# maelaubert/VulkanSift

Hardware: AMD Instinct MI355X
Metric: SIFT detect+match frames/sec (640x480, ~2k kp) (higher is better)
Workload: dtype f32

## Files before the change

### vulkansift_amd/csrc/hip/extract_tail.hip

```cpp
#include <hip/hip_runtime.h>
#include <stdint.h>

#include "extrema_refine.h"
#include "multi.h"
#include "records.h"
#include "vksift_hip.h"
#include "wave.h"

namespace
{

constexpr uint32_t TAIL_SPT = 2;
constexpr uint32_t TAIL_LIST = 4096;

template <bool F16, bool BUF>
__global__ void __launch_bounds__(1024) __attribute__((amdgpu_waves_per_eu(6, 8))) k_extract_tail(Multi<ExtremaArgs> m)
{
  __shared__ uint32_t s_list[TAIL_LIST];
  __shared__ uint32_t s_wtot[2][16];
  __shared__ uint32_t s_cnt[2][16];
  const VBlock vb = vblock(m);
  const ExtremaArgs &a = m.oct[vb.o];
  const int b = (int)vb.x;
  const uint32_t tid = threadIdx.x, NT = blockDim.x, nw = NT >> 6, lane = tid & 63u, wave = tid >> 6;
  constexpr unsigned EB = F16 ? 2u : 4u;
  const DogView d{(const float *)((const uint8_t *)a.gauss + (size_t)b * a.img_stride * EB), a.w, a.h, a.pitch, (size_t)a.plane_stride, a.S};
  const __amdgpu_buffer_rsrc_t rsrc = __builtin_amdgcn_make_buffer_rsrc((void *)d.base, 0, (int)((unsigned)(a.S + 3) * (unsigned)a.plane_stride * EB), 0x00020000);
  const RefineCtx c{a, 0u, 0u, d, rsrc, nullptr, nullptr, nullptr};
  const uint64_t *__restrict__ mask = a.seg_mask + (size_t)b * a.seg_img_stride;
  uint8_t *const feats = a.feats + (size_t)b * a.feat_img_stride;
  const uint32_t nsegs = a.nsegs, tile = NT * TAIL_SPT;

  uint32_t base = 0;
  uint32_t ncand = 0;
  uint32_t fill = 0;
  uint32_t rpar = 0;

  auto round = [&](uint32_t c0, uint32_t cnt) {
    KpRecord kp;
    bool ok = false;
    if (tid < cnt)
      ok = refine_candidate<F16, BUF>(c, s_list[c0 + tid], &kp);
    const unsigned long long bal = __ballot(ok);
    if (lane == 0)
      s_cnt[rpar][wave] = (uint32_t)__popcll(bal);
    __syncthreads();
    uint32_t rank = ballot_rank(bal, (int)lane), total = 0;
    for (uint32_t wv = 0; wv < nw; wv++)
    {
      const uint32_t n = s_cnt[rpar][wv];
      rank += wv < wave ? n : 0u;
      total += n;
    }
    const uint32_t idx = base + rank;
    if (ok && idx < a.cap)
      store_record((uint32_t *)(feats + (size_t)idx * VKSIFT_RECORD_BYTES), kp);
    base += total;
    rpar ^= 1u;
  };

  auto load_tile = [&](uint32_t t0, unsigned long long(&mk)[TAIL_SPT]) {
    const uint32_t i0 = t0 + TAIL_SPT * tid;
#pragma unroll
    for (uint32_t k = 0; k < TAIL_SPT; k++)
      mk[k] = i0 + k < nsegs ? mask[i0 + k] : 0ull;
  };

  unsigned long long cur[TAIL_SPT];
  uint32_t tpar = 0;
  for (uint32_t t0 = 0; t0 < nsegs; t0 += tile, tpar ^= 1u)
  {
    load_tile(t0, cur);
    uint32_t tsum = 0;
#pragma unroll
    for (uint32_t k = 0; k < TAIL_SPT; k++)
      tsum += (uint32_t)__popcll(cur[k]);
    const uint32_t incl = wave_scan_incl_u32(tsum, (int)lane);
    if (lane == 63u)
      s_wtot[tpar][wave] = incl;
    __syncthreads();
    uint32_t off = incl - tsum, T = 0;
    for (uint32_t wv = 0; wv < nw; wv++)
    {
      const uint32_t n = s_wtot[tpar][wv];
      off += wv < wave ? n : 0u;
      T += n;
    }
    const uint32_t valid = ncand >= a.cand_cap ? 0u : (T < a.cand_cap - ncand ? T : a.cand_cap - ncand);
    ncand += T;
    for (uint32_t w0 = 0; w0 < valid;)
    {
      const uint32_t room = TAIL_LIST - fill, hi = valid - w0 < room ? valid : w0 + room;
      if (off < hi && off + tsum > w0)
      {
        uint32_t pos = off;
#pragma unroll
        for (uint32_t k = 0; k < TAIL_SPT; k++)
        {
          unsigned long long mk = cur[k];
          if (mk == 0ull)
            continue;
          const uint32_t seg = t0 + TAIL_SPT * tid + k;
          const uint32_t row = seg / (uint32_t)a.nseg, segx = seg - row * (uint32_t)a.nseg;
          const uint32_t sz = row / (uint32_t)a.h, yy = row - sz * (uint32_t)a.h;
          const uint32_t head = (segx * 64u) | (yy << 14) | ((sz + 1u) << 28);
          while (mk)
          {
            const uint32_t bit = (uint32_t)__ffsll((long long)mk) - 1u;
            mk &= mk - 1ull;
            if (pos >= w0 && pos < hi)
              s_list[fill + (pos - w0)] = head + bit;
            pos++;
          }
        }
      }
      fill += hi - w0;
      w0 = hi;
      __syncthreads();
      const uint32_t nfull = fill - fill % NT, left = fill - nfull;
      for (uint32_t c0 = 0; c0 < nfull; c0 += NT)
        round(c0, NT);
      if (nfull != 0u && left != 0u)
      {
        if (tid < left)
          s_list[tid] = s_list[nfull + tid];
        __syncthreads();
      }
      fill = left;
    }
  }
  if (fill != 0u)
    round(0u, fill);
  if (tid == 0u)
  {
    a.cand_n[b] = ncand;
    a.found[(size_t)b * a.found_img_stride] = base;
  }
}

}

int extract_tail_launch(const ExtremaArgs *args, uint32_t n, uint32_t batch, bool f16, bool buf, bool small_wg, hipStream_t hs)
{
  Multi<ExtremaArgs> mt;
  mt.n = 0;
  for (uint32_t i = 0; i < n; i++)
    if (!multi_add(mt, args[i], batch, 1u, 1u))
      return (int)hipErrorInvalidValue;
  const dim3 grid(mt.start[mt.n]), block(mt.start[mt.n] < 512u && !small_wg ? 1024u : 512u);
  with_bool(f16, [&](auto F16) {
    with_bool(buf, [&](auto BUF) { hipLaunchKernelGGL((k_extract_tail<decltype(F16)::value, decltype(BUF)::value>), grid, block, 0, hs, mt); });
  });
  return (int)hipGetLastError();
}
```

### vulkansift_amd/csrc/hip/extrema.hip

```cpp
#include <hip/hip_runtime.h>
#include <type_traits>
#include <vector>
#include <stdint.h>
#include <stdlib.h>

#include "../detmath.h"
#include "extrema_refine.h"
#include "multi.h"
#include "records.h"
#include "vksift_hip.h"
#include "wave.h"

namespace
{

__device__ __forceinline__ float wave_shr1(float v, float edge)
{
  return __builtin_bit_cast(float, __builtin_amdgcn_update_dpp(__builtin_bit_cast(int, edge), __builtin_bit_cast(int, v), 0x138, 0xf, 0xf, false));
}
__device__ __forceinline__ float wave_shl1(float v, float edge)
{
  return __builtin_bit_cast(float, __builtin_amdgcn_update_dpp(__builtin_bit_cast(int, edge), __builtin_bit_cast(int, v), 0x130, 0xf, 0xf, false));
}

// ... 162 lines not shown
      const float vxh = fmax3(ho, hm, hn), vnh = fmin3(ho, hm, hn);
      const float Lx = wave_shr1(vxb, vxh), Ln = wave_shr1(vnb, vnh);
      const float Rx = wave_shl1(vxa, vxh), Rn = wave_shl1(vna, vnh);
      if (l >= 1 && l <= S)
      {
        ownxA[l - 1] = fmax3(Lx, vxb, fmax2(ao, an)), ownnA[l - 1] = fmin3(Ln, vnb, fmin2(ao, an));
        ownxB[l - 1] = fmax3(vxa, Rx, fmax2(bo, bn)), ownnB[l - 1] = fmin3(vna, Rn, fmin2(bo, bn));
      }
      fullxA[l] = fmax3(Lx, vxa, vxb), fullnA[l] = fmin3(Ln, vna, vnb);
      fullxB[l] = fmax3(vxa, vxb, Rx), fullnB[l] = fmin3(vna, vnb, Rn);
    }
#pragma unroll
    for (int sz = 0; sz < S; sz++)
    {
      const int l = sz + 1;
      const float ca = __uint_as_float(wv2[sm][l].x), cb = __uint_as_float(wv2[sm][l].y);
      const float nxa = fmax3(ownxA[sz], fullxA[l - 1], fullxA[l + 1]), nna = fmin3(ownnA[sz], fullnA[l - 1], fullnA[l + 1]);
      const float nxb = fmax3(ownxB[sz], fullxB[l - 1], fullxB[l + 1]), nnb = fmin3(ownnB[sz], fullnB[l - 1], fullnB[l + 1]);
      const unsigned long long ma = (__ballot(ca > nxa) | __ballot(ca < nna)) & __ballot(fabsf(ca) > pre) & colA;
      const unsigned long long mb = (__ballot(cb > nxb) | __ballot(cb < nnb)) & __ballot(fabsf(cb) > pre) & colB;
      if ((ma | mb) != 0ull)
      {
        const unsigned lo = odd ? (unsigned)mb : (unsigned)ma, hi = odd ? (unsigned)(mb >> 32) : (unsigned)(ma >> 32);
        const unsigned long long m0 = __ballot((lo >> half) & 1u), m1 = __ballot((hi >> half) & 1u);
        if (lane == 0)
        {
          const size_t base = ((size_t)sz * a.h + y) * a.nseg + (size_t)b * a.seg_img_stride;
          a.seg_mask[base + seg0] = m0;
          if (has_seg1)
            a.seg_mask[base + seg0 + 1] = m1;
        }
      }
    }
  };

  if (AHEAD >= 1)
    fetch_row(y0 - 1, std::integral_constant<int, 0>{});
  if (AHEAD >= 2)
    fetch_row(y0, std::integral_constant<int, 1 % NSLOT>{});
  int r = y0 - 1;
  for (;;)
  {
    phase(std::integral_constant<int, 0>{}, r);
    if (++r > y1)
      break;
    phase(std::integral_constant<int, 1>{}, r);
    if (++r > y1)
      break;
    phase(std::integral_constant<int, 2>{}, r);
    if (++r > y1)
      break;
    phase(std::integral_constant<int, 3>{}, r);
    if (++r > y1)
      break;
    if (NSLOT > 4)
    {
      phase(std::integral_constant<int, 4 % NSLOT>{}, r);
      if (++r > y1)
        break;
    }
  }
}

constexpr uint32_t SEG_CHUNK = 4096;

__global__ void __launch_bounds__(1024) k_segment_scan(Multi<ExtremaArgs> m)
{
  __shared__ uint32_t wave_tot[16];
  const VBlock vb = vblock(m);
  const ExtremaArgs &a = m.oct[vb.o];
  const int b = (int)vb.y;
  const uint64_t *__restrict__ mask = a.seg_mask + (size_t)b * a.seg_img_stride;
  uint32_t *__restrict__ off = a.seg_off + (size_t)b * a.seg_img_stride;
  uint32_t *__restrict__ chunk_tot = a.cand_flag;
  const uint64_t chunk_img_stride = a.cand_img_stride;
  const uint32_t n = a.nsegs;
  const int lane = threadIdx.x & 63, wave = threadIdx.x >> 6;
  const uint32_t i0 = vb.x * SEG_CHUNK + 4u * threadIdx.x;
  uint32_t p[4];
#pragma unroll
  for (int k = 0; k < 4; k++)
    p[k] = i0 + k < n ? (uint32_t)__popcll(mask[i0 + k]) : 0u;
  const uint32_t tsum = p[0] + p[1] + p[2] + p[3];
  const uint32_t incl = wave_scan_incl_u32(tsum, lane);
  if (lane == 63)
    wave_tot[wave] = incl;
  __syncthreads();
  uint32_t wave_base = 0, total = 0;
  for (int wv = 0; wv < 16; wv++)
  {
    if (wv < wave)
      wave_base += wave_tot[wv];
    total += wave_tot[wv];
  }
  uint32_t run = wave_base + incl - tsum;
#pragma unroll
  for (int k = 0; k < 4; k++)
  {
    if (i0 + k < n)
      off[i0 + k] = run;
    run += p[k];
  }
  if (threadIdx.x == 0)
    chunk_tot[(size_t)b * chunk_img_stride + vb.x] = total;
}


__global__ void __launch_bounds__(256) k_cand_list(Multi<ExtremaArgs> mu)
{
  const VBlock vb = vblock(mu);
  const ExtremaArgs &a = mu.oct[vb.o];
  const uint32_t seg = vb.x * 256 + threadIdx.x;
  const int b = (int)vb.y;
  const uint32_t *chunk_tot = a.cand_flag + (size_t)b * a.cand_img_stride;
  if (vb.x == 0 && threadIdx.x == 0)
  {
    uint32_t total = 0;
    for (uint32_t c = 0; c < a.nchunks; c++)
      total += chunk_tot[c];
    a.cand_n[b] = total;
    if (total == 0)
      a.found[(size_t)b * a.found_img_stride] = 0;
  }
  unsigned long long m = seg < a.nsegs ? a.seg_mask[seg + (size_t)b * a.seg_img_stride] : 0ull;
  if (__ballot(m != 0ull) == 0ull)
    return;
  uint32_t base = 0;
  for (uint32_t c = threadIdx.x & 63u, nc = (vb.x * 256u) / SEG_CHUNK; c < nc; c += 64u)
    base += chunk_tot[c];
  base = wave_sum_u32(base);
  if (m == 0ull)
    return;
  uint32_t pos = a.seg_off[seg + (size_t)b * a.seg_img_stride] + base;
  const uint32_t segx = seg % (uint32_t)a.nseg;
  const uint32_t yy = (seg / (uint32_t)a.nseg) % (uint32_t)a.h;
  const uint32_t sz = seg / ((uint32_t)a.nseg * (uint32_t)a.h);
  uint32_t *out = a.cand_xy + (size_t)b * a.cand_img_stride;
  while (m)
  {
    const int bit = __ffsll((long long)m) - 1;
    m &= m - 1;
    if (pos < a.cand_cap)
      out[pos] = (segx * 64u + (uint32_t)bit) | (yy << 14) | ((sz + 1u) << 28);
    pos++;
  }
}

template <bool F16, bool BUF>
__global__ void __launch_bounds__(256) k_refine_flags(Multi<ExtremaArgs> m)
{
  __shared__ uint32_t s_cnt[4];
  const VBlock vb = vblock(m);
  const RefineCtx c = refine_ctx<F16>(m.oct[vb.o], (int)vb.x);
  for (uint32_t chunk = vb.y; chunk < c.nch; chunk += vb.gy)
  {
    const uint32_t i = chunk * 256u + threadIdx.x;
    bool ok = false;
    if (i < c.n)
    {
      KpRecord kp;
      ok = refine_candidate<F16, BUF>(c, c.xy[i], &kp);
      c.flag[i] = ok ? 1u : 0u;
    }
    const unsigned long long bal = __ballot(ok);
    if ((threadIdx.x & 63) == 0)
      s_cnt[threadIdx.x >> 6] = (uint32_t)__popcll(bal);
    __syncthreads();
// ... 229 lines not shown
```

### vulkansift_amd/csrc/hip/features.hip

```cpp
#include <hip/hip_runtime.h>
#include <stdint.h>
#include <stdlib.h>
#include <type_traits>

#include "../detmath.h"
#include "features_math.h"
#include "multi.h"
#include "records.h"
#include "vksift_hip.h"
#include "wave.h"

namespace
{

struct FeatArgs
{
  const float *gauss;
  uint32_t fp16;
  int w, h, pitch;
  uint64_t plane_stride, img_stride;
  uint8_t *feats;
  uint64_t feat_img_stride;
  uint32_t cap;
  uint32_t *found;
// ... 128 lines not shown
            px -= box, py++;
          const float sdx = (rsx + (float)dx) - kh.scale_x;
          const float sdy = (rsy + (float)dy) - kh.scale_y;
          const float d2 = (sdx * sdx) + (sdy * sdy);
          if constexpr (decltype(INTERIOR)::value)
          {
            const unsigned v0 = (__umul24((unsigned)(cyi + dy - 1), (unsigned)g.pitch) + (unsigned)(cxi + dx - 1)) * 4u;
            accumulate(d2, tap_ld<F16>(kh.rs, v0 + 8u, pitch4), tap_ld<F16>(kh.rs, v0, pitch4), tap_ld<F16>(kh.rs, v0 + 4u, 2 * pitch4), tap_ld<F16>(kh.rs, v0 + 4u, 0));
          }
          else
          {
            const int gx = cxi + dx, gy = cyi + dy;
            if ((gx < 1 || gx >= (g.w - 1) || gy < 1 || gy >= (g.h - 1)) && (d2 > (float)(r * r)))
              continue;
            const bool xin = (unsigned)gx < (unsigned)g.w, yin = (unsigned)gy < (unsigned)g.h;
            const unsigned o0 = (__umul24((unsigned)gy, (unsigned)g.pitch) + (unsigned)gx) * 4u;
            const unsigned o_r = (yin && (unsigned)(gx + 1) < (unsigned)g.w) ? o0 + 4u : 0x80000000u;
            const unsigned o_l = (yin && (unsigned)(gx - 1) < (unsigned)g.w) ? o0 - 4u : 0x80000000u;
            const unsigned o_d = (xin && (unsigned)(gy + 1) < (unsigned)g.h) ? (__umul24((unsigned)(gy + 1), (unsigned)g.pitch) + (unsigned)gx) * 4u : 0x80000000u;
            const unsigned o_u = (xin && (unsigned)(gy - 1) < (unsigned)g.h) ? (__umul24((unsigned)(gy - 1), (unsigned)g.pitch) + (unsigned)gx) * 4u : 0x80000000u;
            accumulate(d2, tap_ld<F16>(kh.rs, o_r, 0), tap_ld<F16>(kh.rs, o_l, 0), tap_ld<F16>(kh.rs, o_d, 0), tap_ld<F16>(kh.rs, o_u, 0));
          }
        }
      };
      if (cxi - r >= 1 && cxi + r <= g.w - 2 && cyi - r >= 1 && cyi + r <= g.h - 2)
        window(std::true_type{});
      else
        window(std::false_type{});
    }
    __builtin_amdgcn_wave_barrier();
    {
      const int li = lane < 36 ? lane : 0;
      uint32_t hv = hist[li];
      const int lm = (li + 35) % 36, lp = (li + 1) % 36;
#pragma unroll
      for (int it = 0; it < 6; it++)
      {
        uint32_t hm = __shfl(hv, lm, 64), hp = __shfl(hv, lp, 64);
        hv = (uint32_t)dm_div_3((float)(hm + hv + hp));
      }
      uint32_t hm = __shfl(hv, lm, 64), hp = __shfl(hv, lp, 64);
      const uint32_t mx = wave_max_u32(lane < 36 ? hv : 0u);
      bool peak = lane < 36 && ((float)hv >= (0.8f * (float)mx)) && (hv > hm) && (hv > hp);
      unsigned long long pm = __ballot(peak);
      uint32_t npk = (uint32_t)__popcll(pm);
      if (peak)
      {
        uint32_t rank = ballot_rank(pm, lane);
        if (rank < a.max_keep)
        {
          uint32_t num = hm - hp;
          uint32_t den = hm - (2u * hv) + hp;
          float idx = (float)lane + 0.5f * ((float)num / (float)den);
          float ang = (idx + 0.5f) * (2.f * PI_F) / 36.f;
          a.ori_ang[((size_t)b * a.ori_img_stride + k) * VKSIFT_HIP_MAX_ORI + rank] = ang;
        }
      }
      if (lane == 0)
        a.ori_cnt[(size_t)b * a.ori_img_stride + k] = npk < a.max_keep ? npk : a.max_keep;
    }
    __builtin_amdgcn_wave_barrier();
  }
}

__global__ void __launch_bounds__(1024) k_orientation_finalize(Multi<FeatArgs> m)
{
  __shared__ uint32_t wave_tot[16];
  __shared__ uint32_t carry_s;
  const VBlock vb = vblock(m);
  const FeatArgs &a = m.oct[vb.o];
  const int b = (int)vb.x;
  const int lane = threadIdx.x & 63, wave = threadIdx.x >> 6;
  const ImageView g = image_view(a, b);
  const uint32_t *cnt = a.ori_cnt + (size_t)b * a.ori_img_stride;
  const float *ang = a.ori_ang + (size_t)b * a.ori_img_stride * VKSIFT_HIP_MAX_ORI;
  if (threadIdx.x == 0)
    carry_s = 0;
  __syncthreads();
  for (uint32_t base = 0; base < g.n; base += 1024)
  {
    uint32_t k = base + threadIdx.x;
    uint32_t c = k < g.n ? cnt[k] : 0u;
    uint32_t v = c > 1 ? c - 1 : 0u;
    const uint32_t incl = wave_scan_incl_u32(v, lane);
    if (lane == 63)
      wave_tot[wave] = incl;
    __syncthreads();
    uint32_t wave_base = 0;
    for (int wv = 0; wv < wave; wv++)
      wave_base += wave_tot[wv];
    uint32_t carry = carry_s;
    uint32_t excl = carry + wave_base + incl - v;
    if (k < g.n && c >= 1)
    {
      uint32_t *rec = (uint32_t *)(g.feats + (size_t)k * VKSIFT_RECORD_BYTES);
      rec[7] = __float_as_uint(ang[(size_t)k * VKSIFT_HIP_MAX_ORI]);
      for (uint32_t j = 1; j < c; j++)
      {
        uint32_t idx = g.found + excl + (j - 1);
        if (idx < a.cap)
        {
          uint32_t *dst = (uint32_t *)(g.feats + (size_t)idx * VKSIFT_RECORD_BYTES);
#pragma unroll
          for (int q = 0; q < (int)VKSIFT_RECORD_HEAD_WORDS; q++)
            dst[q] = rec[q];
          dst[7] = __float_as_uint(ang[(size_t)k * VKSIFT_HIP_MAX_ORI + j]);
        }
      }
    }
    __syncthreads();
    if (threadIdx.x == 1023)
      carry_s = carry + wave_base + incl;
    __syncthreads();
  }
  if (threadIdx.x == 0)
    a.found[(size_t)b * a.found_img_stride] = g.found + carry_s;
}

__device__ __forceinline__ int smod8(int v) { return v & 7; }

struct DescCtx
{
  __amdgpu_buffer_rsrc_t rs;
  int pitch, pitch4;
  float scale_x, scale_y, rsx, rsy, kcos, ksin, kori, fp, bin_scale;
  int dx0, dx1, dy0, dy1;
  float offx, offy, ia0, ia1;
};

struct DescSample
{
  float ox, oy, mag;
  float xb;
};

struct DescTaps
{
  float up, lf, rt, dn;
};

__device__ __forceinline__ unsigned desc_tap_base(const DescCtx &c, int cdx, int cdy)
{
  const int ix = (int)c.rsx + cdx, iy = (int)c.rsy + cdy;
  return (__umul24((unsigned)(iy - 1), (unsigned)c.pitch) + (unsigned)(ix - 1)) * 4u;
}

template <bool F16>
__device__ __forceinline__ DescTaps desc_taps(const DescCtx &c, unsigned v0)
{
  DescTaps t;
  t.up = tap_ld<F16>(c.rs, v0 + 4u, 0);
  t.lf = tap_ld<F16>(c.rs, v0, c.pitch4);
  t.rt = tap_ld<F16>(c.rs, v0 + 8u, c.pitch4);
  t.dn = tap_ld<F16>(c.rs, v0 + 4u, 2 * c.pitch4);
  return t;
}

typedef uint32_t u32x2_t __attribute__((ext_vector_type(2)));
typedef uint32_t u32x4_t __attribute__((ext_vector_type(4)));
__device__ __forceinline__ void desc_taps_pair(const DescCtx &c, unsigned v0, DescTaps &a, DescTaps &b)
{
  const u32x2_t up = __builtin_amdgcn_raw_buffer_load_b64(c.rs, v0 + 4u, 0, 0);
  const u32x4_t mid = __builtin_amdgcn_raw_buffer_load_b128(c.rs, v0, c.pitch4, 0);
  const u32x2_t dn = __builtin_amdgcn_raw_buffer_load_b64(c.rs, v0 + 4u, 2 * c.pitch4, 0);
  a.up = __uint_as_float(up.x), b.up = __uint_as_float(up.y);
  a.lf = __uint_as_float(mid.x), b.lf = __uint_as_float(mid.y);
  a.rt = __uint_as_float(mid.z), b.rt = __uint_as_float(mid.w);
  a.dn = __uint_as_float(dn.x), b.dn = __uint_as_float(dn.y);
}

template <bool INRANGE>
__device__ __forceinline__ DescSample desc_sample(const DescCtx &c, int cdx, int cdy, const DescTaps &t, bool *odd)
{
  const float es = -1.f / (2.f * 2 * 2);
  float sdx = (c.rsx + (float)cdx) - c.scale_x;
  float sdy = (c.rsy + (float)cdy) - c.scale_y;
  DescSample r;
  r.ox = c.kcos * sdx + c.ksin * sdy;
  r.oy = c.kcos * sdy - c.ksin * sdx;
  float gradX = 0.5f * (t.rt - t.lf);
  float gradY = 0.5f * (t.dn - t.up);
  float ori, root;
  grad_polar<INRANGE>(gradX, gradY, &ori, &root, odd);
  ori = wrap_2pi(ori);
  ori = wrap_2pi(ori - c.kori);
  r.mag = dm_expf_core_nonpos(es * ((r.ox * r.ox) + (r.oy * r.oy))) * root;
  r.xb = ori * c.bin_scale;
  return r;
}

constexpr int DESC_PAD = 1, DESC_ROW_CELLS = 8;
constexpr int DESC_HIST_WORDS = (4 + 2 * DESC_PAD) * DESC_ROW_CELLS * 16;
constexpr int DESC_WORK_WORDS = DESC_HIST_WORDS;
__device__ __forceinline__ int desc_cell_word(int cell)
{
  return (((cell >> 2) + DESC_PAD) * DESC_ROW_CELLS + (cell & 3) + DESC_PAD) * 16;
}
__device__ __forceinline__ uint32_t desc_hist_read(const uint32_t *s_work, int t)
{
  const int cw = desc_cell_word(t >> 3), bin = t & 7;
  return s_work[cw + 2 * bin] + s_work[cw + 2 * ((bin + 7) & 7) + 1];
}

__device__ __forceinline__ void desc_scatter(const DescCtx &c, const DescSample &r, float fbin, bool live, uint32_t *s_work)
{
  float fhx = r.ox + 2.f, fhy = r.oy + 2.f;
  const float flx = floorf(fhx - 0.5f), fly = floorf(fhy - 0.5f), flb = floorf(fbin);
  int hx = (int)flx, hy = (int)fly, hb = (int)flb;
  float rhx = fhx - (flx + 0.5f), rhy = fhy - (fly + 0.5f), rb = fbin - flb;
  const float magfp = r.mag * c.fp;
  const unsigned b0 = (unsigned)smod8(hb);
  const unsigned pair = b0 * 8u;
  const bool okx[2] = {live && (unsigned)hx < 4u, live && (unsigned)(hx + 1) < 4u};
  const bool oky[2] = {(unsigned)hy < 4u, (unsigned)(hy + 1) < 4u};
  char *base = (char *)s_work + ((unsigned)((hy + DESC_PAD) * (DESC_ROW_CELLS * 64) + (hx + DESC_PAD) * 64) + pair);
#pragma unroll
  for (int i = 0; i < 2; i++)
#pragma unroll
    for (int j = 0; j < 2; j++)
    {
      const float w = fabsf(1.f - (float)i - rhx) * fabsf(1.f - (float)j - rhy);
      const uint32_t v0 = (uint32_t)((w * fabsf(1.f - 0.f - rb)) * magfp);
      const uint32_t v1 = (uint32_t)((w * fabsf(1.f - 1.f - rb)) * magfp);
      if (okx[i] && oky[j])
        atomicAdd((unsigned long long *)(base + (j * DESC_ROW_CELLS * 64 + i * 64)), ((unsigned long long)v1 << 32) | v0);
    }
}

constexpr int DESC_MAX_ROWS = 256;

template <bool CAN_POST>
__device__ __forceinline__ void desc_dense_prologue(const FeatArgs &a, const vksift_hip_DenseRows &dr, int b, bool first_block, int tid, uint32_t *s_row0)
{
  if (!(dr.desc || (CAN_POST && dr.post)))
    return;
  const uint32_t *fsec = a.found + (size_t)b * a.found_img_stride - a.sec;
  uint32_t row0 = 0, total = 0;
#pragma unroll
  for (uint32_t j = 0; j < 16u; j++)
    if (j < dr.nsec)
    {
      const uint32_t f = fsec[j], n = f < dr.sec_cap[j] ? f : dr.sec_cap[j];
      row0 += j < a.sec ? n : 0u;
      total += n;
    }
  if (tid == 0)
    *s_row0 = row0;
  if (a.sec == 0 && first_block)
  {
    if (CAN_POST && dr.post && (uint32_t)tid < dr.found_post_n)
      dr.found_post[(size_t)b * dr.found_post_n + tid] = fsec[tid];
    if (dr.desc && tid == 0)
      dr.n[(size_t)b * dr.n_img_stride] = total;
    if (dr.desc && total < 2u && tid < 64)
    {
      uint32_t *z = (uint32_t *)(dr.desc + (size_t)b * dr.desc_img_stride);
      if (tid >= (int)total * 32)
        z[tid] = 0u;
      if (tid < 2 && tid >= (int)total)
        dr.norm[(size_t)b * dr.norm_img_stride + tid] = 128u * 128u * 128u;
    }
  }
}

__device__ __forceinline__ DescCtx desc_setup(const FeatArgs &a, const ImageView &g, const KeyHead &kh)
{
  DescCtx c;
  c.scale_x = kh.scale_x, c.scale_y = kh.scale_y, c.kori = kh.theta;
  c.rs = kh.rs;
  c.pitch = g.pitch, c.pitch4 = g.pitch * 4;
  c.bin_scale = a.use_vlfeat ? 8.f : -8.f;
  float scale_factor = dm_pow2i(kh.octave_idx);
  float lambda = 3.0f * (kh.sigma / scale_factor);
  float radius = sqrtf(2.f) * lambda * 5.f * 0.5f;
  int R = (int)floorf(radius + 0.5f);
  float sn, cs;
  dm_sincosf(c.kori, &sn, &cs);
  c.kcos = cs / lambda, c.ksin = sn / lambda;
  uint32_t ti = (uint32_t)(R / 2);
  c.fp = a.desc_fp_tab[ti < a.desc_fp_tab_len ? ti : a.desc_fp_tab_len - 1];
  c.rsx = roundf(c.scale_x), c.rsy = roundf(c.scale_y);

  const int cxi = (int)c.rsx, cyi = (int)c.rsy;
  c.dx0 = max(-R, 1 - cxi), c.dx1 = min(R, g.w - 2 - cxi);
  c.dy0 = max(-R, 1 - cyi), c.dy1 = min(R, g.h - 2 - cyi);
  c.offx = c.rsx - c.scale_x, c.offy = c.rsy - c.scale_y;
  c.ia0 = __builtin_amdgcn_rcpf(c.kcos), c.ia1 = __builtin_amdgcn_rcpf(-c.ksin);
  return c;
}

struct DescRows
{
  int *lo;
  uint32_t *cnt;
  const uint32_t *pre;
  int y0, nrows;
};

template <int NT>
__device__ __forceinline__ void desc_row_spans(const DescCtx &c, const DescRows &rows, int tid)
{
  const float T = 2.5f + 0.01f;
  for (int row = tid; row < rows.nrows; row += NT)
  {
    const float fy = (float)(rows.y0 + row) + c.offy;
    float lo = (float)c.dx0 - 0.5f, hi = (float)c.dx1 + 0.5f;
#pragma unroll
    for (int e = 0; e < 2; e++)
    {
      const float aa = e == 0 ? c.kcos : -c.ksin, ia = e == 0 ? c.ia0 : c.ia1;
      const float bb = e == 0 ? c.ksin * fy : c.kcos * fy;
      if (fabsf(aa) > 1e-12f)
      {
        const float ctr = -bb * ia - c.offx, half = T * fabsf(ia);
        lo = fmaxf(lo, ctr - half);
        hi = fminf(hi, ctr + half);
      }
      else if (!(fabsf(bb) < T))
        hi = lo - 2.f;
    }
    const int ilo = (int)ceilf(lo - 0.01f), ihi = (int)floorf(hi + 0.01f);
    const int xl = max(ilo, c.dx0), xh = min(ihi, c.dx1);
    rows.lo[row] = xl;
    rows.cnt[row] = xh >= xl ? (uint32_t)(xh - xl + 1) : 0u;
  }
}

__device__ __forceinline__ void desc_row_prefix(const DescRows &rows, uint32_t *pre, int lane)
{
  uint32_t carry = 0;
  for (int base = 0; base < rows.nrows; base += 64)
  {
    const int i = base + lane;
    const uint32_t v = i < rows.nrows ? rows.cnt[i] : 0u;
    const uint32_t incl = wave_scan_incl_u32(v, lane);
    if (i < rows.nrows)
      pre[i] = carry + incl - v;
    carry += __shfl(incl, 63, 64);
  }
  if (lane == 0)
    pre[rows.nrows] = carry;
}

struct DescRun
{
  uint32_t steps;
  uint32_t sidx, send;
  int row, cdx;
  uint32_t row_end;
};
template <int NWV>
__device__ __forceinline__ DescRun desc_run(const DescRows &rows, int wave, int lane)
{
  const uint32_t *s_pre = rows.pre;
  const uint32_t N = s_pre[rows.nrows];
  const uint32_t T = (N + 63u) / 64u, tq = T / NWV, tr = T % NWV;
  DescRun r;
  r.steps = tq + ((uint32_t)wave < tr ? 1u : 0u);
  const uint32_t step0 = (uint32_t)wave * tq + min((uint32_t)wave, tr);
  r.sidx = min(N, step0 * 64u + (uint32_t)lane * r.steps);
  r.send = min(N, r.sidx + r.steps);
  int row = 0;
  if (r.sidx < r.send)
  {
    int lo_r = 0, hi_r = rows.nrows - 1;
    while (lo_r < hi_r)
    {
      const int mid = (lo_r + hi_r + 1) >> 1;
      if (s_pre[mid] <= r.sidx)
        lo_r = mid;
      else
        hi_r = mid - 1;
    }
    row = lo_r;
    while (s_pre[row + 1] <= r.sidx)
      row++;
  }
  r.row = row;
  r.cdx = rows.lo[row] + (int)(r.sidx - s_pre[row]);
  r.row_end = s_pre[row + 1];
  return r;
}

__device__ __forceinline__ bool desc_next_sample(const DescRows &rows, DescRun &r, int &sx, int &sy)
{
  const bool live = r.sidx < r.send;
  if (live && r.sidx >= r.row_end)
  {
    do
      r.row++;
    while (rows.pre[r.row + 1] <= r.sidx);
    r.row_end = rows.pre[r.row + 1];
    r.cdx = rows.lo[r.row];
  }
  sx = r.cdx, sy = rows.y0 + r.row;
  r.cdx++, r.sidx++;
  return live;
}

template <bool F16>
__device__ __forceinline__ void desc_step_pair(const DescCtx &c, const DescRows &rows, DescRun &run, uint32_t *s_work)
{
  int sx[2], sy[2];
  const bool live[2] = {desc_next_sample(rows, run, sx[0], sy[0]), desc_next_sample(rows, run, sx[1], sy[1])};
  DescTaps t0, t1;
  const unsigned v0 = desc_tap_base(c, sx[0], sy[0]);
  if (F16)
  {
    t0 = desc_taps<F16>(c, v0);
    t1 = desc_taps<F16>(c, desc_tap_base(c, sx[1], sy[1]));
  }
  else
  {
    desc_taps_pair(c, v0, t0, t1);
    if (live[1] && !(sy[1] == sy[0] && sx[1] == sx[0] + 1))
      t1 = desc_taps<F16>(c, desc_tap_base(c, sx[1], sy[1]));
  }
  bool o0, o1;
// ... 129 lines not shown
      for (; it + 1 < run.steps; it += 2)
        desc_step_pair<F16>(c, rows, run, s_work);
      if (it < run.steps)
        desc_step_odd<F16>(c, rows, run, s_work);
    }
    __syncthreads();
    if (wave == 0)
      desc_epilogue<CAN_POST>(dr, g, b, k, kh.rec, s_work, &s_row0, lane);
  }
}

FeatArgs make_args(const vksift_hip_OctaveJob *job)
{
  FeatArgs a;
  a.gauss = job->gauss;
  a.fp16 = job->fp16;
  a.w = (int)job->w, a.h = (int)job->h, a.pitch = (int)job->pitch;
  a.plane_stride = job->plane_stride, a.img_stride = job->img_stride;
  a.feats = job->feats, a.feat_img_stride = job->feat_img_stride, a.cap = job->cap;
  a.found = job->found, a.found_img_stride = job->found_img_stride;
  a.ori_ang = job->ori_ang, a.ori_cnt = job->ori_cnt, a.ori_img_stride = job->ori_img_stride;
  uint32_t mk = job->max_ori == 0 ? VKSIFT_HIP_MAX_ORI : job->max_ori;
  a.max_keep = mk > VKSIFT_HIP_MAX_ORI ? VKSIFT_HIP_MAX_ORI : mk;
  a.use_vlfeat = job->use_vlfeat;
  a.desc_fp_tab = job->desc_fp_tab, a.desc_fp_tab_len = job->desc_fp_tab_len;
  a.sec = job->sec_index;
  return a;
}

bool img_fast(uint32_t batch, bool descriptor)
{
  return batch > 1 && !descriptor;
}

bool add_octave(Multi<FeatArgs> &m, const FeatArgs &a, bool img_fast, uint32_t batch, uint32_t blocks)
{
  return multi_add(m, a, img_fast ? batch : blocks, img_fast ? blocks : batch, 1u);
}

uint32_t expected_keypoints(const vksift_hip_OctaveJob *job, uint32_t batch)
{
  const uint32_t pixels_per_keypoint = 512;
  if (batch < 8u)
    return 0xFFFFFFFFu;
  const uint64_t n = (uint64_t)job->w * job->h / pixels_per_keypoint;
  return n < 32u ? 32u : (n > 0xFFFFFFFFull ? 0xFFFFFFFFu : (uint32_t)n);
}

uint32_t octave_blocks(const vksift_hip_OctaveJob *job, uint32_t batch, uint32_t kp_per_block, uint32_t cap_blocks)
{
  const uint32_t dense = expected_keypoints(job, batch);
  uint32_t blocks = ((job->cap < dense ? job->cap : dense) + (kp_per_block - 1)) / kp_per_block;
  if (blocks > cap_blocks)
    blocks = cap_blocks;
  return blocks == 0 ? 1 : blocks;
}

}

static int orientation_run(const vksift_hip_OctaveJob *jobs, uint32_t n, uint32_t batch, hipStream_t hs)
{
  Multi<FeatArgs> mo, mf;
  mo.n = mf.n = 0;
  const bool f = img_fast(batch, false);
  uint32_t cap_blocks = 16384u / batch;
  cap_blocks = cap_blocks < 32u ? 32u : (cap_blocks > 1024u ? 1024u : cap_blocks);
  for (uint32_t i = 0; i < n; i++)
  {
    const FeatArgs a = make_args(&jobs[i]);
    if (!add_octave(mo, a, f, batch, octave_blocks(&jobs[i], batch, 4, cap_blocks)) || !multi_add(mf, a, batch, 1u, 1u))
      return (int)hipErrorInvalidValue;
  }
  const bool f16 = mo.oct[0].fp16 != 0;
  const dim3 grid(mo.start[mo.n]);
  with_bool(f, [&](auto IMG_FAST) {
    with_bool(f16, [&](auto F16) { hipLaunchKernelGGL((k_orientation<decltype(IMG_FAST)::value, decltype(F16)::value>), grid, dim3(256), 0, hs, mo); });
  });
  hipLaunchKernelGGL(k_orientation_finalize, dim3(mf.start[mf.n]), dim3(1024), 0, hs, mf);
  return (int)hipGetLastError();
}

static int descriptor_run(const vksift_hip_OctaveJob *jobs, uint32_t n, uint32_t batch, const vksift_hip_DenseRows &dr, hipStream_t hs)
{
  Multi<FeatArgs> md;
  md.n = 0;
  const bool f = img_fast(batch, true);
  for (uint32_t i = 0; i < n; i++)
    if (!add_octave(md, make_args(&jobs[i]), f, batch, octave_blocks(&jobs[i], batch, 1, 2048)))
      return (int)hipErrorInvalidValue;
  const bool two_waves = batch >= 8u;
  if (dr.post && two_waves)
    return (int)hipErrorInvalidValue;
  const bool f16 = md.oct[0].fp16 != 0;
  const dim3 grid(md.start[md.n]);
  with_bool(two_waves, [&](auto TWO) {
    constexpr int NWV = decltype(TWO)::value ? 2 : 4;
    with_bool(f, [&](auto IMG_FAST) {
      with_bool(f16, [&](auto F16) {
        hipLaunchKernelGGL((k_descriptor<NWV, decltype(IMG_FAST)::value, decltype(F16)::value>), grid, dim3(64 * NWV), 0, hs, md, dr);
      });
    });
  });
  return (int)hipGetLastError();
}

template <typename F>
static int for_runs(const vksift_hip_OctaveJob *jobs, uint32_t n_jobs, F run)
{
  for (uint32_t i0 = 0; i0 < n_jobs;)
  {
    uint32_t i1 = i0 + 1;
    while (i1 < n_jobs && i1 - i0 < multi_run_max() && jobs[i1].fp16 == jobs[i0].fp16)
      i1++;
    const int e = run(jobs + i0, i1 - i0);
    if (e)
      return e;
    i0 = i1;
  }
  return 0;
}

extern "C"
{
  int vksift_hip_orientations_multi(const vksift_hip_OctaveJob *jobs, uint32_t n_jobs, uint32_t batch, vksift_hip_stream s)
  {
    if (batch == 0)
      return 0;
    return for_runs(jobs, n_jobs, [&](const vksift_hip_OctaveJob *j, uint32_t n) { return orientation_run(j, n, batch, (hipStream_t)s); });
  }

  int vksift_hip_descriptors_multi_dense(const vksift_hip_OctaveJob *jobs, uint32_t n_jobs, uint32_t batch, const vksift_hip_DenseRows *dense,
                                         vksift_hip_stream s)
  {
    if (batch == 0)
      return 0;
    vksift_hip_DenseRows dr = {};
    if (dense)
    {
      const bool rows = dense->desc != NULL, post = dense->post != NULL;
      if ((!rows && !post) || (rows && (!dense->norm || !dense->n)) || (post && (!dense->found_post || dense->found_post_n > 64u)) || dense->nsec == 0 ||
          dense->nsec > 16u)
        return (int)hipErrorInvalidValue;
      for (uint32_t i = 0; i < n_jobs; i++)
        if (jobs[i].sec_index >= dense->nsec)
          return (int)hipErrorInvalidValue;
      dr = *dense;
    }
    return for_runs(jobs, n_jobs, [&](const vksift_hip_OctaveJob *j, uint32_t n) { return descriptor_run(j, n, batch, dr, (hipStream_t)s); });
  }

  int vksift_hip_descriptors_multi(const vksift_hip_OctaveJob *jobs, uint32_t n_jobs, uint32_t batch, vksift_hip_stream s)
  {
    return vksift_hip_descriptors_multi_dense(jobs, n_jobs, batch, nullptr, s);
  }

  int vksift_hip_orientations(const vksift_hip_OctaveJob *job, uint32_t batch, vksift_hip_stream s) { return vksift_hip_orientations_multi(job, 1, batch, s); }

  int vksift_hip_descriptors(const vksift_hip_OctaveJob *job, uint32_t batch, vksift_hip_stream s) { return vksift_hip_descriptors_multi(job, 1, batch, s); }
}
```

### vulkansift_amd/csrc/hip/strongest.hip

```cpp
#include <hip/hip_runtime.h>
#include <stdint.h>

#include "vksift_hip.h"
#include "hip/records.h"
#include "hip/wave.h"

#define STRONGEST_LDS_KEYS 8192u
#define STRONGEST_KEY_WORD 8u

namespace
{

__global__ void __launch_bounds__(1024) k_keep_strongest(uint32_t *__restrict__ feats_base, uint64_t buf_stride, GatherMap map, SectionTable tab,
                                                         uint32_t *__restrict__ found_base, uint32_t found_buf_stride, uint32_t *__restrict__ found_post,
                                                         uint32_t max_features, CacheEntry cache)
{
  __shared__ uint32_t off_s[VKSIFT_MAX_SECTIONS], cnt_s[VKSIFT_MAX_SECTIONS], kept_s[VKSIFT_MAX_SECTIONS];
  __shared__ uint32_t hist[256], keys_s[STRONGEST_LDS_KEYS];
  __shared__ uint32_t wave_tot[16], tie_carry, keep_carry, sel_s[2];
  const uint32_t tid = threadIdx.x, lane = tid & 63u;
  const uint32_t bufi = map.buf[blockIdx.x];
  const auto buf = buffer_ref(feats_base, buf_stride, found_base, found_buf_stride, bufi);
  uint32_t *const feats = buf.recs, *const found = buf.found;

  if (tid < VKSIFT_MAX_SECTIONS)
  {
    const uint32_t raw = tid < tab.nsec ? raw_count(tab, found, tid) : 0u;
    off_s[tid] = tab.off[tid];
    cnt_s[tid] = section_stored(raw, tab.cap[tid]);
    kept_s[tid] = 0;
  }
  if (tid == 0)
    tie_carry = 0, keep_carry = 0;
  __syncthreads();
  uint32_t cnt[VKSIFT_MAX_SECTIONS];
  const uint32_t total = section_counts(VKSIFT_MAX_SECTIONS, [&](uint32_t o) { return cnt_s[o]; }, cnt_s, cnt);
  if (total <= max_features)
    return;

  auto key_at = [&](uint32_t row) { return feats[(size_t)section_row(cnt, off_s, row) * VKSIFT_RECORD_WORDS + STRONGEST_KEY_WORD] & 0x7FFFFFFFu; };

  uint32_t prefix = 0, want = max_features;
  for (uint32_t pass = 0; pass < 4u; pass++)
  {
    const uint32_t shift = 24u - 8u * pass, decided = pass ? 0xFFFFFFFFu << (shift + 8u) : 0u;
    if (tid < 256u)
      hist[tid] = 0;
    __syncthreads();
    for (uint32_t row = tid; row < total; row += 1024u)
    {
      uint32_t key;
      if (pass == 0u)
      {
        key = key_at(row);
        if (row < STRONGEST_LDS_KEYS)
          keys_s[row] = key;
      }
      else
        key = row < STRONGEST_LDS_KEYS ? keys_s[row] : key_at(row);
      if ((key & decided) == prefix)
        atomicAdd(&hist[(key >> shift) & 255u], 1u);
    }
    __syncthreads();
    if (tid < 64u)
    {
      uint32_t h[4], sum = 0;
      for (uint32_t i = 0; i < 4u; i++)
        h[i] = hist[255u - 4u * tid - i], sum += h[i];
      const uint32_t incl = wave_scan_incl_u32(sum, (int)lane);
      uint32_t above = incl - sum;
      if (above < want && want <= incl)
      {
        uint32_t bin = 255u - 4u * tid;
        for (uint32_t i = 0; i < 3u && want > above + h[i]; i++)
          above += h[i], bin--;
        sel_s[0] = bin, sel_s[1] = want - above;
      }
    }
    __syncthreads();
    prefix |= sel_s[0] << shift;
    want = sel_s[1];
  }
  const uint32_t threshold = prefix, quota = want;

  const CacheEntry entry = cache_entry_of(cache, bufi);
  for (uint32_t base = 0; base < total; base += 1024u)
  {
    const uint32_t row = base + tid;
    uint32_t key = 0, sec = 0, src_row = 0;
    const bool valid = row < total;
    if (valid)
    {
      key = row < STRONGEST_LDS_KEYS ? keys_s[row] : key_at(row);
      src_row = section_row(cnt, off_s, row);
      uint32_t first = 0;
      VKSIFT_UNROLL
      for (uint32_t o = 0; o < VKSIFT_MAX_SECTIONS; o++)
      {
        if (row >= first && row < first + cnt[o])
          sec = o;
        first += cnt[o];
      }
    }
    const bool tie = valid && key == threshold;
    const uint32_t tie_rank = ordered_keep(tie, wave_tot, tie_carry);
    const bool keep = valid && (key > threshold || (tie && tie_rank < quota));
    const uint32_t out_row = ordered_keep(keep, wave_tot, keep_carry);
    VKSIFT_UNROLL
    for (uint32_t o = 0; o < VKSIFT_MAX_SECTIONS; o++)
    {
      const unsigned long long bal = __ballot(keep && sec == o);
      if (lane == 0u && bal)
        atomicAdd(&kept_s[o], (uint32_t)__popcll(bal));
    }
    __syncthreads();
    uint32_t rec[VKSIFT_RECORD_WORDS], dst_row = 0;
    if (keep)
    {
      uint32_t in_front = 0;
      VKSIFT_UNROLL
      for (uint32_t o = 0; o < VKSIFT_MAX_SECTIONS; o++)
        in_front += o < sec ? kept_s[o] : 0u;
      dst_row = off_s[sec] + (out_row - in_front);
      const uint32_t *src = feats + (size_t)src_row * VKSIFT_RECORD_WORDS;
      VKSIFT_UNROLL
      for (uint32_t w = 0; w < VKSIFT_RECORD_WORDS; w++)
        rec[w] = src[w];
    }
    __builtin_amdgcn_s_waitcnt(0);
    __syncthreads();
    if (keep)
    {
      if (dst_row != src_row)
      {
        uint32_t *dst = feats + (size_t)dst_row * VKSIFT_RECORD_WORDS;
        VKSIFT_UNROLL
        for (uint32_t w = 0; w < VKSIFT_RECORD_WORDS; w++)
          dst[w] = rec[w];
      }
      if (entry.rows && out_row < max_features)
      {
        uint32_t norm = 0;
        VKSIFT_UNROLL
        for (uint32_t q = 0; q < 8u; q++)
        {
          const uint32_t *d = rec + VKSIFT_RECORD_HEAD_WORDS + 4u * q;
          const uint4 v = uint4{d[0], d[1], d[2], d[3]};
          *(uint4 *)(entry.rows + (size_t)out_row * 32u + 4u * q) = v;
          norm += shifted_norm_part(v);
        }
        entry.norms[out_row] = norm;
      }
// ... 39 lines not shown
```

### vulkansift_amd/csrc/hip/wave.h

```cpp
#pragma once
#include <hip/hip_runtime.h>
#include <stdint.h>

template <int LANES> __device__ __forceinline__ uint32_t lanes_sum_u32(uint32_t v)
{
#pragma unroll
  for (int dlt = LANES / 2; dlt >= 1; dlt >>= 1)
    v += __shfl_xor(v, dlt, 64);
  return v;
}

__device__ __forceinline__ uint32_t wave_sum_u32(uint32_t v) { return lanes_sum_u32<64>(v); }

__device__ __forceinline__ uint32_t wave_max_u32(uint32_t v)
{
#pragma unroll
  for (int dlt = 32; dlt >= 1; dlt >>= 1)
  {
    const uint32_t t = __shfl_xor(v, dlt, 64);
    v = t > v ? t : v;
  }
  return v;
}

__device__ __forceinline__ uint32_t wave_scan_incl_u32(uint32_t v, int lane)
{
#pragma unroll
  for (int dlt = 1; dlt < 64; dlt <<= 1)
  {
    const uint32_t t = __shfl_up(v, dlt, 64);
    if (lane >= dlt)
      v += t;
  }
  return v;
}

__device__ __forceinline__ uint32_t ballot_rank(unsigned long long bal, int lane) { return (uint32_t)__popcll(bal & ((1ull << lane) - 1ull)); }
```

Measured before the change: 26040.

## Precompute descriptor constants in a prepass kernel and use a DPP wave scan

Adds a small kernel that computes each keypoint's descriptor setup constants (rotation, bounds, offsets, reciprocals) once. It stores them in the record's descriptor field, where the descriptor kernel reads them back through constant-address-space scalar loads instead of recomputing them in every wave. Separately, the inclusive wave scan now uses DPP row shifts and row broadcasts instead of shfl_up loops, and every scan call site drops the lane argument. The cost is an extra kernel launch and extra global traffic. It also relies on the descriptor kernel reading these constants before it overwrites the field, and on the record pointer being wave-uniform.

```diff
diff --git a/vulkansift_amd/csrc/hip/extract_tail.hip b/vulkansift_amd/csrc/hip/extract_tail.hip
--- a/vulkansift_amd/csrc/hip/extract_tail.hip
+++ b/vulkansift_amd/csrc/hip/extract_tail.hip
@@ -75,7 +75,7 @@
 #pragma unroll
     for (uint32_t k = 0; k < TAIL_SPT; k++)
       tsum += (uint32_t)__popcll(cur[k]);
-    const uint32_t incl = wave_scan_incl_u32(tsum, (int)lane);
+    const uint32_t incl = wave_scan_incl_u32(tsum);
     if (lane == 63u)
       s_wtot[tpar][wave] = incl;
     __syncthreads();
diff --git a/vulkansift_amd/csrc/hip/extrema.hip b/vulkansift_amd/csrc/hip/extrema.hip
--- a/vulkansift_amd/csrc/hip/extrema.hip
+++ b/vulkansift_amd/csrc/hip/extrema.hip
@@ -268,7 +268,7 @@
   for (int k = 0; k < 4; k++)
     p[k] = i0 + k < n ? (uint32_t)__popcll(mask[i0 + k]) : 0u;
   const uint32_t tsum = p[0] + p[1] + p[2] + p[3];
-  const uint32_t incl = wave_scan_incl_u32(tsum, lane);
+  const uint32_t incl = wave_scan_incl_u32(tsum);
   if (lane == 63)
     wave_tot[wave] = incl;
   __syncthreads();
diff --git a/vulkansift_amd/csrc/hip/features.hip b/vulkansift_amd/csrc/hip/features.hip
--- a/vulkansift_amd/csrc/hip/features.hip
+++ b/vulkansift_amd/csrc/hip/features.hip
@@ -234,7 +234,7 @@
     uint32_t k = base + threadIdx.x;
     uint32_t c = k < g.n ? cnt[k] : 0u;
     uint32_t v = c > 1 ? c - 1 : 0u;
-    const uint32_t incl = wave_scan_incl_u32(v, lane);
+    const uint32_t incl = wave_scan_incl_u32(v);
     if (lane == 63)
       wave_tot[wave] = incl;
     __syncthreads();
@@ -271,13 +271,20 @@
 
 __device__ __forceinline__ int smod8(int v) { return v & 7; }
 
-struct DescCtx
+struct DescConsts
+{
+  float kcos, ksin, kori, fp, rsx, rsy, scale_x, scale_y;
+  int dx0, dx1, dy0, dy1;
+  float offx, offy, ia0, ia1;
+};
+constexpr int DESC_CONST_WORDS = 16;
+static_assert(sizeof(DescConsts) == DESC_CONST_WORDS * 4 && DESC_CONST_WORDS * 4 <= (int)(VKSIFT_RECORD_BYTES - VKSIFT_RECORD_DESC_AT), "the constants fit the descriptor field");
+
+struct DescCtx : DescConsts
 {
   __amdgpu_buffer_rsrc_t rs;
   int pitch, pitch4;
-  float scale_x, scale_y, rsx, rsy, kcos, ksin, kori, fp, bin_scale;
-  int dx0, dx1, dy0, dy1;
-  float offx, offy, ia0, ia1;
+  float bin_scale;
 };
 
 struct DescSample
@@ -415,15 +422,14 @@
   }
 }
 
-__device__ __forceinline__ DescCtx desc_setup(const FeatArgs &a, const ImageView &g, const KeyHead &kh)
-{
-  DescCtx c;
-  c.scale_x = kh.scale_x, c.scale_y = kh.scale_y, c.kori = kh.theta;
-  c.rs = kh.rs;
-  c.pitch = g.pitch, c.pitch4 = g.pitch * 4;
-  c.bin_scale = a.use_vlfeat ? 8.f : -8.f;
-  float scale_factor = dm_pow2i(kh.octave_idx);
-  float lambda = 3.0f * (kh.sigma / scale_factor);
+__device__ __forceinline__ DescConsts desc_ctx_compute(const FeatArgs &a, const ImageView &g, const float *rec)
+{
+  DescConsts c;
+  c.scale_x = rec[2], c.scale_y = rec[3], c.kori = rec[7];
+  const int octave_idx = ((const int *)rec)[5];
+  const float sigma = rec[6];
+  float scale_factor = dm_pow2i(octave_idx);
+  float lambda = 3.0f * (sigma / scale_factor);
   float radius = sqrtf(2.f) * lambda * 5.f * 0.5f;
   int R = (int)floorf(radius + 0.5f);
   float sn, cs;
@@ -438,6 +444,41 @@
   c.dy0 = max(-R, 1 - cyi), c.dy1 = min(R, g.h - 2 - cyi);
   c.offx = c.rsx - c.scale_x, c.offy = c.rsy - c.scale_y;
   c.ia0 = __builtin_amdgcn_rcpf(c.kcos), c.ia1 = __builtin_amdgcn_rcpf(-c.ksin);
+  return c;
+}
+
+__global__ void __launch_bounds__(256) k_descriptor_consts(Multi<FeatArgs> m)
+{
+  const VBlock vb = vblock(m);
+  const FeatArgs &a = m.oct[vb.o];
+  const int b = (int)vb.y;
+  const ImageView g = image_view(a, b);
+  for (uint32_t k = vb.x * 256u + threadIdx.x; k < g.n; k += vb.gx * 256u)
+  {
+    float *rec = (float *)(g.feats + (size_t)k * VKSIFT_RECORD_BYTES);
+    const DescConsts c = desc_ctx_compute(a, g, rec);
+    uint32_t w[DESC_CONST_WORDS];
+    __builtin_memcpy(w, &c, sizeof(c));
+    uint32_t *dst = (uint32_t *)rec + VKSIFT_RECORD_HEAD_WORDS;
+#pragma unroll
+    for (int q = 0; q < DESC_CONST_WORDS; q++)
+      dst[q] = w[q];
+  }
+}
+
+typedef const uint32_t __attribute__((address_space(4))) *ConstWords;
+__device__ __forceinline__ DescCtx desc_setup(const FeatArgs &a, const ImageView &g, const KeyHead &kh)
+{
+  DescCtx c;
+  const ConstWords p = (ConstWords)(uintptr_t)(kh.rec + VKSIFT_RECORD_HEAD_WORDS);
+  uint32_t w[DESC_CONST_WORDS];
+#pragma unroll
+  for (int q = 0; q < DESC_CONST_WORDS; q++)
+    w[q] = p[q];
+  __builtin_memcpy(static_cast<DescConsts *>(&c), w, sizeof(DescConsts));
+  c.rs = kh.rs;
+  c.pitch = g.pitch, c.pitch4 = g.pitch * 4;
+  c.bin_scale = a.use_vlfeat ? 8.f : -8.f;
   return c;
 }
 
@@ -485,7 +526,7 @@
   {
     const int i = base + lane;
     const uint32_t v = i < rows.nrows ? rows.cnt[i] : 0u;
-    const uint32_t incl = wave_scan_incl_u32(v, lane);
+    const uint32_t incl = wave_scan_incl_u32(v);
     if (i < rows.nrows)
       pre[i] = carry + incl - v;
     carry += __shfl(incl, 63, 64);
@@ -781,17 +822,21 @@
 
 static int descriptor_run(const vksift_hip_OctaveJob *jobs, uint32_t n, uint32_t batch, const vksift_hip_DenseRows &dr, hipStream_t hs)
 {
-  Multi<FeatArgs> md;
-  md.n = 0;
+  Multi<FeatArgs> md, mc;
+  md.n = mc.n = 0;
   const bool f = img_fast(batch, true);
   for (uint32_t i = 0; i < n; i++)
-    if (!add_octave(md, make_args(&jobs[i]), f, batch, octave_blocks(&jobs[i], batch, 1, 2048)))
+  {
+    const FeatArgs a = make_args(&jobs[i]);
+    if (!add_octave(md, a, f, batch, octave_blocks(&jobs[i], batch, 1, 2048)) || !multi_add(mc, a, octave_blocks(&jobs[i], batch, 256, 16), batch, 1u))
       return (int)hipErrorInvalidValue;
+  }
   const bool two_waves = batch >= 8u;
   if (dr.post && two_waves)
     return (int)hipErrorInvalidValue;
   const bool f16 = md.oct[0].fp16 != 0;
   const dim3 grid(md.start[md.n]);
+  hipLaunchKernelGGL(k_descriptor_consts, dim3(mc.start[mc.n]), dim3(256), 0, hs, mc);
   with_bool(two_waves, [&](auto TWO) {
     constexpr int NWV = decltype(TWO)::value ? 2 : 4;
     with_bool(f, [&](auto IMG_FAST) {
diff --git a/vulkansift_amd/csrc/hip/strongest.hip b/vulkansift_amd/csrc/hip/strongest.hip
--- a/vulkansift_amd/csrc/hip/strongest.hip
+++ b/vulkansift_amd/csrc/hip/strongest.hip
@@ -67,7 +67,7 @@
       uint32_t h[4], sum = 0;
       for (uint32_t i = 0; i < 4u; i++)
         h[i] = hist[255u - 4u * tid - i], sum += h[i];
-      const uint32_t incl = wave_scan_incl_u32(sum, (int)lane);
+      const uint32_t incl = wave_scan_incl_u32(sum);
       uint32_t above = incl - sum;
       if (above < want && want <= incl)
       {
diff --git a/vulkansift_amd/csrc/hip/wave.h b/vulkansift_amd/csrc/hip/wave.h
--- a/vulkansift_amd/csrc/hip/wave.h
+++ b/vulkansift_amd/csrc/hip/wave.h
@@ -23,15 +23,18 @@
   return v;
 }
 
-__device__ __forceinline__ uint32_t wave_scan_incl_u32(uint32_t v, int lane)
+template <int CTRL, int ROW_MASK> __device__ __forceinline__ uint32_t dpp_or_zero(uint32_t v)
 {
-#pragma unroll
-  for (int dlt = 1; dlt < 64; dlt <<= 1)
-  {
-    const uint32_t t = __shfl_up(v, dlt, 64);
-    if (lane >= dlt)
-      v += t;
-  }
+  return (uint32_t)__builtin_amdgcn_update_dpp(0, (int)v, CTRL, ROW_MASK, 0xf, true);
+}
+__device__ __forceinline__ uint32_t wave_scan_incl_u32(uint32_t v)
+{
+  v += dpp_or_zero<0x111, 0xf>(v);
+  v += dpp_or_zero<0x112, 0xf>(v);
+  v += dpp_or_zero<0x114, 0xf>(v);
+  v += dpp_or_zero<0x118, 0xf>(v);
+  v += dpp_or_zero<0x142, 0xa>(v);
+  v += dpp_or_zero<0x143, 0xc>(v);
   return v;
 }
 
```

Result: no change. 26190, median of 6 (+0.6%).
